# miemie2013/Pytorch-PPYOLO

Measured on AMD Instinct MI355X. Metric: images/sec PPYOLO R50-vd 608x608 bs=8, higher is better.
Workload: dtype f32; 1 GPU; PPYOLO ResNet50-vd (DCNv2, CoordConv, SPP) 608x608, 8 images per GPU, device-resident input -> padded detections; global_batch=8, parallelism=single GPU, hip_graph=True, tile_table=tuned_gfx950_f16x2.json

## Files before the change

### pytorch-ppyolo_amd/ppyolo_hip/csrc/conv_patch.hip

```cpp
#include "conv_shared.h"
#pragma clang fp contract(off)

#ifndef PPY_PATCH_ABL
#define PPY_PATCH_ABL 0
#endif

namespace {

constexpr unsigned PT_OOB = 0x80000000u;
constexpr int PT_TH = 8, PT_TW = 32, PT_PW = PT_TW + 2, PT_NPIX = (PT_TH + 2) * PT_PW;
constexpr int PT_PLANE = PT_NPIX * 64;
constexpr int PT_UNITS = PT_NPIX * 8, PT_NST = (PT_UNITS + 511) / 512;

constexpr int PM_ROWS = 3, PM_COLS = 15;

struct PatchArgs {
    ConvArgs c;
    int tiles_x, tiles_y, ntiles;
    int Hp, Wp;
};

template <int TN, bool BNS = false, bool MPOOL = false>
__global__ void __launch_bounds__(512, 1) conv3x3_patch_kernel(const PatchArgs q) {
    static_assert(!(BNS && MPOOL), "statistics of a tensor that is not stored");
    static_assert(PT_TH * PM_COLS * 32 * TN * 4 <= 2 * PT_PLANE, "the x-pooled rows fit the operand planes");
#if defined(__HIP_DEVICE_COMPILE__)
    const ConvArgs &p = q.c;
    constexpr int K = 32 * TN, WBYTES = 9 * 2 * K * 64;
    extern __shared__ __attribute__((aligned(16))) char smem_pt[];
    char *pl_hi = smem_pt, *pl_lo = smem_pt + PT_PLANE, *wl = smem_pt + 2 * PT_PLANE;
    const int tid = threadIdx.x, lane = tid & 63;
    const int wave = __builtin_amdgcn_readfirstlane(tid >> 6);
    float *sE = reinterpret_cast<float *>(smem_pt + 2 * PT_PLANE + WBYTES) + wave * (32 * LDS_LD);
    const __amdgpu_buffer_rsrc_t rx = __builtin_amdgcn_make_buffer_rsrc((void *)p.x, 0, PT_OOB, 0x00020000);
    const __amdgpu_buffer_rsrc_t ry = __builtin_amdgcn_make_buffer_rsrc((void *)p.y, 0, PT_OOB, 0x00020000);

    {
        const char *wb = reinterpret_cast<const char *>(p.wf16);
        const long long plane_bytes = (long long)K * 9 * 32 * 2;
        constexpr int WUNITS = 9 * 2 * K * 4, NWL = (WUNITS + 511) / 512;
        uintx4 wv[NWL];
#pragma unroll
        for (int i = 0; i < NWL; ++i) {
            const int u = min(tid + 512 * i, WUNITS - 1);
            const int slot = u & 3, row = u >> 2;
            const int k = row % K, tp = row / K, plane = tp & 1, tap = tp >> 1;
            wv[i] = *reinterpret_cast<const uintx4 *>(wb + plane * plane_bytes + ((long long)(tap * K + k) * 32) * 2 + slot * 16);
        }
#pragma unroll
        for (int i = 0; i < NWL; ++i) {
            const int u = tid + 512 * i;
            const int slot = u & 3, row = u >> 2;
            const int k = row % K;
            if (u < WUNITS) *reinterpret_cast<uintx4 *>(wl + row * 64 + ((slot ^ ((k >> 2) & 3)) << 4)) = wv[i];
        }
    }
    const int erow = lane >> 3, ec4 = (lane & 7) * 4;
    floatx4 sc[TN], sh[TN];
#pragma unroll
    for (int j = 0; j < TN; ++j) {
        sc[j] = *reinterpret_cast<const floatx4 *>(p.scale + j * 32 + ec4);
        sh[j] = *reinterpret_cast<const floatx4 *>(p.shift + j * 32 + ec4);
    }
#pragma unroll
    for (int j = 0; j < TN; ++j) asm volatile("" : "+v"(sc[j]), "+v"(sh[j]));

    int s_py[PT_NST], s_px[PT_NST];
#pragma unroll
    for (int i = 0; i < PT_NST; ++i) {
        const int pp = min((tid + 512 * i) >> 3, PT_NPIX - 1);
        s_py[i] = pp / PT_PW;
        s_px[i] = pp - s_py[i] * PT_PW;
    }
    uintx4 stg_a[PT_NST], stg_b[PT_NST];
#pragma unroll
    for (int i = 0; i < PT_NST; ++i) stg_a[i] = stg_b[i] = uintx4{0u, 0u, 0u, 0u};
    const int tiles_img = q.tiles_x * q.tiles_y;
    auto tile_of = [&](int t, int &n, int &y0, int &x0) {
        n = t / tiles_img;
        const int r = t - n * tiles_img, by = r / q.tiles_x;
        y0 = MPOOL ? 2 * PM_ROWS * by - 1 : by * PT_TH;
        x0 = MPOOL ? 2 * PM_COLS * (r - by * q.tiles_x) - 1 : (r - by * q.tiles_x) * PT_TW;
    };
    auto request = [&](int t, uintx4 (&stg)[PT_NST]) {
        int n, y0, x0;
        tile_of(max(t, 0), n, y0, x0);
        const bool live = t >= 0 && t < q.ntiles;
#pragma unroll
        for (int i = 0; i < PT_NST; ++i) {
            const int y = y0 - 1 + s_py[i], x = x0 - 1 + s_px[i];
            const bool ok = live && tid + 512 * i < PT_UNITS && (unsigned)y < (unsigned)p.H && (unsigned)x < (unsigned)p.W;
            const unsigned off = ok ? (unsigned)((n * p.H + y) * p.W + x) * (unsigned)(p.x_ld * 4) + (unsigned)((tid + 512 * i) & 7) * 16u : PT_OOB;
            if (PPY_PATCH_ABL != 4) stg[i] = __builtin_amdgcn_raw_buffer_load_b128(rx, (int)off, 0, 0);
        }
    };

    int sc_n = -1;
    float sa = 1.f, inv_sa = 1.f;
    int run_n = -1;
    float run_mx = 0.f;
    auto flush = [&](float mx, int n) {
        if (p.amax_out && n >= 0) {
#pragma unroll
            for (int o = 32; o > 0; o >>= 1) mx = fmaxf(mx, __shfl_xor(mx, o));
            if (lane == 0) amax_store(mx, p.amax_out, n, (int)blockIdx.x * 8 + wave);
        }
    };
    const float slope = p.act == PPY_ACT_RELU ? 0.f : (p.act == PPY_ACT_LEAKY ? 0.1f : 1.f);
    __syncthreads();
    const int stride = (int)gridDim.x;
    auto do_tile = [&](int t, uintx4 (&stg)[PT_NST]) {
        const bool live = t >= 0 && t < q.ntiles;
        int n, y0, x0;
        tile_of(live ? t : 0, n, y0, x0);
        if (live) {
        if (n != sc_n) {
            const float mx = conv_amax_in(p, n);
            const int e = (int)((__float_as_uint(mx) >> 23) & 0xffu);
            int f = 267 - e;
            f = f < 103 ? 103 : (f > 167 ? 167 : f);
            sa = __uint_as_float((unsigned)f << 23);
            inv_sa = __uint_as_float((unsigned)(254 - f) << 23);
            sc_n = n;
        }
        if (n != run_n) {
            flush(run_mx, run_n);
            run_n = n;
            run_mx = 0.f;
        }
#pragma unroll
        for (int i = 0; i < PT_NST; ++i) {
            const int u = tid + 512 * i;
            if (u < PT_UNITS && PPY_PATCH_ABL != 2) {
                const int pp = u >> 3, g = u & 7;
                const float x0f = __uint_as_float(stg[i][0]), x1f = __uint_as_float(stg[i][1]);
                const float x2f = __uint_as_float(stg[i][2]), x3f = __uint_as_float(stg[i][3]);
                const unsigned h0 = cvt_pk_f16(x0f * sa, x1f * sa), h1 = cvt_pk_f16(x2f * sa, x3f * sa);
                const unsigned l0 = cvt_pk_f16(fmaf(x0f, sa, -f16_lo(h0)), fmaf(x1f, sa, -f16_hi(h0)));
                const unsigned l1 = cvt_pk_f16(fmaf(x2f, sa, -f16_lo(h1)), fmaf(x3f, sa, -f16_hi(h1)));
                const int o = pp * 64 + (((g >> 1) ^ ((pp >> 2) & 3)) << 4) + (g & 1) * 8;
                typedef __attribute__((ext_vector_type(2))) unsigned uintx2;
                *reinterpret_cast<uintx2 *>(pl_hi + o) = uintx2{h0, h1};
                *reinterpret_cast<uintx2 *>(pl_lo + o) = uintx2{l0, l1};
            }
        }
        }
        asm volatile("s_waitcnt lgkmcnt(0)" ::: "memory");
        __builtin_amdgcn_s_barrier();
        request(t + 2 * stride, stg);

        floatx16 acc[TN];
#pragma unroll
        for (int j = 0; j < TN; ++j)
#pragma unroll
            for (int e = 0; e < 16; ++e) acc[j][e] = 0.f;
        const int tx = lane & 31, kh = lane >> 5;
        if (live && PPY_PATCH_ABL != 1 && (!MPOOL || wave < 2 * PM_ROWS + 1)) {
            struct Frag {
                uintx4 a0, a1, b0[TN], b1[TN];
            };
            Frag f[2];
            auto fetch = [&](Frag &fr, int g) {
                const int tap = g >> 1, s2 = g & 1;
                const int pp = (wave + tap / 3) * PT_PW + tx + tap % 3;
                const int ao = pp * 64 + (((2 * s2 + kh) ^ ((pp >> 2) & 3)) << 4);
                fr.a0 = *reinterpret_cast<const uintx4 *>(pl_hi + ao);
                fr.a1 = *reinterpret_cast<const uintx4 *>(pl_lo + ao);
#pragma unroll
                for (int j = 0; j < TN; ++j) {
                    const int k = j * 32 + tx;
                    const int bo = (((2 * s2 + kh) ^ ((k >> 2) & 3)) << 4);
                    fr.b0[j] = *reinterpret_cast<const uintx4 *>(wl + ((tap * 2 + 0) * K + k) * 64 + bo);
                    fr.b1[j] = *reinterpret_cast<const uintx4 *>(wl + ((tap * 2 + 1) * K + k) * 64 + bo);
                }
            };
            fetch(f[0], 0);
#pragma unroll
            for (int g = 0; g < 18; ++g) {
                if (g + 1 < 18 && PPY_PATCH_ABL != 5) fetch(f[(g + 1) & 1], g + 1);
                __builtin_amdgcn_sched_barrier(0);
                const Frag &c = f[PPY_PATCH_ABL == 5 ? 0 : g & 1];
#pragma unroll
                for (int j = 0; j < TN; ++j)
                    acc[j] = __builtin_amdgcn_mfma_f32_32x32x16_f16(__builtin_bit_cast(f16x8, c.a1), __builtin_bit_cast(f16x8, c.b0[j]), acc[j], 0, 0, 0);
#pragma unroll
                for (int j = 0; j < TN; ++j)
                    acc[j] = __builtin_amdgcn_mfma_f32_32x32x16_f16(__builtin_bit_cast(f16x8, c.a0), __builtin_bit_cast(f16x8, c.b1[j]), acc[j], 0, 0, 0);
#pragma unroll
                for (int j = 0; j < TN; ++j)
                    acc[j] = __builtin_amdgcn_mfma_f32_32x32x16_f16(__builtin_bit_cast(f16x8, c.a0), __builtin_bit_cast(f16x8, c.b0[j]), acc[j], 0, 0, 0);
                __builtin_amdgcn_sched_barrier(0);
            }
        }
        asm volatile("s_waitcnt lgkmcnt(0)" ::: "memory");
        __builtin_amdgcn_s_barrier();
        if (!live || PPY_PATCH_ABL == 3) return;

        const int y = y0 + wave;
        const bool row_ok = (unsigned)y < (unsigned)p.H;
        if constexpr (MPOOL) {
            float *xp = reinterpret_cast<float *>(smem_pt);
            constexpr int K4 = K / 4;
            if (wave < 2 * PM_ROWS + 1) {
#pragma unroll
                for (int j = 0; j < TN; ++j) {
#pragma unroll
                    for (int e = 0; e < 16; ++e) {
                        const int row = (e & 3) + 8 * (e >> 2) + 4 * (lane >> 5);
                        sE[row * LDS_LD + (lane & 31)] = acc[j][e];
                    }
                    __builtin_amdgcn_wave_barrier();
#pragma unroll
                    for (int u = 0; u < 4; ++u) {
                        floatx4 v = *reinterpret_cast<const floatx4 *>(sE + (erow + 8 * u) * LDS_LD + ec4);
#pragma unroll
                        for (int c = 0; c < 4; ++c) {
                            const float o = fmaf(v[c] * inv_sa, sc[j][c], sh[j][c]);
                            v[c] = o > 0.f ? o : o * slope + 0.0f;
                        }
                        const bool ok = row_ok && (unsigned)(x0 + erow + 8 * u) < (unsigned)p.W;
                        const float rmx = fmaxf(fmaxf(fabsf(v[0]), fabsf(v[1])), fmaxf(fabsf(v[2]), fabsf(v[3])));
                        run_mx = fmaxf(run_mx, ok ? rmx : 0.f);
                        if (!ok) v = floatx4{-3.402823466e38f, -3.402823466e38f, -3.402823466e38f, -3.402823466e38f};
                        *reinterpret_cast<floatx4 *>(sE + (erow + 8 * u) * LDS_LD + ec4) = v;
                    }
                    __builtin_amdgcn_wave_barrier();
#pragma unroll
                    for (int h = 0; h < 2; ++h) {
                        const int jx = erow + 8 * h;
                        if (jx < PM_COLS) {
                            const floatx4 a = *reinterpret_cast<const floatx4 *>(sE + (2 * jx) * LDS_LD + ec4);
                            const floatx4 b = *reinterpret_cast<const floatx4 *>(sE + (2 * jx + 1) * LDS_LD + ec4);
                            const floatx4 c = *reinterpret_cast<const floatx4 *>(sE + (2 * jx + 2) * LDS_LD + ec4);
                            floatx4 m;
#pragma unroll
                            for (int k = 0; k < 4; ++k) m[k] = fmaxf(fmaxf(a[k], b[k]), c[k]);
                            *reinterpret_cast<floatx4 *>(xp + (wave * PM_COLS + jx) * K + j * 32 + ec4) = m;
                        }
                    }
                    __builtin_amdgcn_wave_barrier();
                }
            }
            asm volatile("s_waitcnt lgkmcnt(0)" ::: "memory");
            __builtin_amdgcn_s_barrier();
            const int by = (y0 + 1) / (2 * PM_ROWS), bx = (x0 + 1) / (2 * PM_COLS);
#pragma unroll
            for (int it = 0; it < (PM_ROWS * PM_COLS * K4 + 511) / 512; ++it) {
                const int i = tid + 512 * it;
                const int r = i / (PM_COLS * K4), rem = i - r * (PM_COLS * K4);
                const int jx = rem / K4, c4 = rem - jx * K4;
                const int py = PM_ROWS * by + r, px = PM_COLS * bx + jx;
                const bool ok = i < PM_ROWS * PM_COLS * K4 && py < q.Hp && px < q.Wp;
                const int rr = ok ? r : 0, jj = ok ? jx : 0;
                const floatx4 a = *reinterpret_cast<const floatx4 *>(xp + ((2 * rr) * PM_COLS + jj) * K + c4 * 4);
                const floatx4 b = *reinterpret_cast<const floatx4 *>(xp + ((2 * rr + 1) * PM_COLS + jj) * K + c4 * 4);
                const floatx4 c = *reinterpret_cast<const floatx4 *>(xp + ((2 * rr + 2) * PM_COLS + jj) * K + c4 * 4);
                floatx4 m;
#pragma unroll
                for (int k = 0; k < 4; ++k) m[k] = fmaxf(fmaxf(a[k], b[k]), c[k]);
                const unsigned off = ok ? (unsigned)((n * q.Hp + py) * q.Wp + px) * (unsigned)(p.y_ld * 4) + (unsigned)c4 * 16u : PT_OOB;
                __builtin_amdgcn_raw_buffer_store_b128(__builtin_bit_cast(uintx4, m), ry, (int)off, 0, 0);
            }
            asm volatile("s_waitcnt lgkmcnt(0)" ::: "memory");
            __builtin_amdgcn_s_barrier();
            return;
        }
        if constexpr (BNS) {
            const int nv = row_ok ? min(max(p.W - x0, 0), 32) : 0;
            const float inv_f[1] = {inv_sa};
            tile_bn_stats<1, TN, 32, 32 * TN>(p, reinterpret_cast<const floatx16(&)[1][TN]>(acc), inv_f, p.M - nv, 0, 0, 0, lane, t * PT_TH + wave);
        }
        const unsigned rowbase = (unsigned)((n * p.H + y) * p.W + x0) * (unsigned)(p.y_ld * 4);
#pragma unroll
        for (int j = 0; j < TN; ++j) {
#pragma unroll
            for (int e = 0; e < 16; ++e) {
                const int row = (e & 3) + 8 * (e >> 2) + 4 * (lane >> 5);
                sE[row * LDS_LD + (lane & 31)] = acc[j][e];
            }
            __builtin_amdgcn_wave_barrier();
#pragma unroll
            for (int u = 0; u < 4; ++u) {
                floatx4 v = *reinterpret_cast<const floatx4 *>(sE + (erow + 8 * u) * LDS_LD + ec4);
#pragma unroll
                for (int c = 0; c < 4; ++c) {
                    const float o = fmaf(v[c] * inv_sa, sc[j][c], sh[j][c]);
                    v[c] = o > 0.f ? o : o * slope + 0.0f;
                }
                const bool ok = row_ok && x0 + erow + 8 * u < p.W;
                const float rmx = fmaxf(fmaxf(fabsf(v[0]), fabsf(v[1])), fmaxf(fabsf(v[2]), fabsf(v[3])));
                run_mx = fmaxf(run_mx, ok ? rmx : 0.f);
                const unsigned off = ok ? rowbase + (unsigned)(erow + 8 * u) * (unsigned)(p.y_ld * 4) + (unsigned)(j * 32 + ec4) * 4u : PT_OOB;
                __builtin_amdgcn_raw_buffer_store_b128(__builtin_bit_cast(uintx4, v), ry, (int)off, 0, 0);
            }
            __builtin_amdgcn_wave_barrier();
        }
    };
    for (int t = (int)blockIdx.x - 2 * stride; t < q.ntiles; t += 2 * stride) {
        do_tile(t, stg_a);
        do_tile(t + stride, stg_b);
    }
    flush(run_mx, run_n);
#endif
}

template <int TN, bool BNS = false, bool MPOOL = false>
int launch_patch(const PatchArgs &q, hipStream_t stream) {
    if constexpr (!BNS && !MPOOL) {
        if (q.c.bn_part) return launch_patch<TN, true>(q, stream);
    }
    auto k = conv3x3_patch_kernel<TN, BNS, MPOOL>;
    const size_t lds = (size_t)2 * PT_PLANE + (size_t)9 * 2 * 32 * TN * 64 + (size_t)8 * 32 * LDS_LD * sizeof(float);
    static PpyLdsAttr attr;
    if (ppy_lds_attr(attr, reinterpret_cast<const void *>(k), (int)lds) != PPY_OK) return PPY_ERR_LAUNCH;
    const int grid = q.ntiles < 256 ? q.ntiles : 256;
    hipLaunchKernelGGL(k, dim3(grid), dim3(512), lds, stream, q);
    return ppy_launch_status();
}

}

int ppy_patch_num_configs() { return 1; }

int ppy_patch_config_info(int local, ppy_conv_cfg_info *out) {
    if (local != 0) return PPY_ERR_BAD_ARG;
    *out = ppy_cfg_info(PPY_CFG_PATCH, local, PPY_CFG_OPERANDS_F16X2, 0, 0, 0, PPY_CFG_SPLITK_NONE, false, false, true);
    return PPY_OK;
}

int ppy_patch_dispatch(const ConvArgs &p, int local, hipStream_t stream) {
    if (local != 0) return PPY_ERR_BAD_ARG;
    if (p.R != 3 || p.S != 3 || p.stride != 1 || p.pad != 1 || p.C != 32 || (p.K != 32 && p.K != 64) || p.ups || p.posb || p.res)
        return PPY_ERR_BAD_ARG;
    if (!p.wf16 || ((uintptr_t)p.wf16 & 15) != 0 || !p.scale_f16 || !p.amax_in) return PPY_ERR_BAD_ARG;
    if (!vec_epilogue_ok(p) || ((uintptr_t)p.x & 15) != 0 || p.x_ld % 4 != 0) return PPY_ERR_BAD_ARG;
    const long long lim = 0x7FFFF000LL;
    if ((long long)p.M * p.x_ld * 4 >= lim || (long long)p.M * p.y_ld * 4 >= lim) return PPY_ERR_UNSUPPORTED;
    if (p.bn_part) {
        if (p.act != PPY_ACT_NONE) return PPY_ERR_UNSUPPORTED;
        if (p.N * ceil_div(p.W, PT_TW) * ceil_div(p.H, PT_TH) * PT_TH > p.bn_capacity) return PPY_ERR_WORKSPACE;
        if (p.bn_slices_host) *p.bn_slices_host = p.N * ceil_div(p.W, PT_TW) * ceil_div(p.H, PT_TH) * PT_TH;
    }
    PatchArgs q;
    q.c = p;
    q.c.scale = p.scale_f16;
    q.Hp = q.Wp = 0;
    q.tiles_x = ceil_div(p.W, PT_TW);
    q.tiles_y = ceil_div(p.H, PT_TH);
    q.ntiles = p.N * q.tiles_x * q.tiles_y;
    return p.K == 32 ? launch_patch<1>(q, stream) : launch_patch<2>(q, stream);
}

int ppy_patch_maxpool_dispatch(const ConvArgs &p, int Hp, int Wp, hipStream_t stream) {
    if (p.R != 3 || p.S != 3 || p.stride != 1 || p.pad != 1 || p.C != 32 || p.K != 64 || p.ups || p.posb || p.res || p.bn_part || p.xscale || p.yscale)
        return PPY_ERR_BAD_ARG;
    if (!p.wf16 || ((uintptr_t)p.wf16 & 15) != 0 || !p.scale_f16 || !p.amax_in) return PPY_ERR_BAD_ARG;
    if (((uintptr_t)p.x & 15) != 0 || p.x_ld % 4 != 0 || ((uintptr_t)p.y & 15) != 0 || p.y_ld % 4 != 0) return PPY_ERR_BAD_ARG;
    if (Hp != (p.H - 1) / 2 + 1 || Wp != (p.W - 1) / 2 + 1) return PPY_ERR_BAD_ARG;
    const long long lim = 0x7FFFF000LL;
    if ((long long)p.M * p.x_ld * 4 >= lim || (long long)p.N * Hp * Wp * p.y_ld * 4 >= lim) return PPY_ERR_UNSUPPORTED;
    PatchArgs q;
    q.c = p;
    q.c.scale = p.scale_f16;
    q.Hp = Hp;
    q.Wp = Wp;
    q.tiles_x = ceil_div(Wp, PM_COLS);
    q.tiles_y = ceil_div(Hp, PM_ROWS);
    q.ntiles = p.N * q.tiles_x * q.tiles_y;
    return launch_patch<2, false, true>(q, stream);
}
```

Before: 2465 images/s.

## Carry last conv row between pooled tiles to drop halo recompute in conv+maxpool

The fused 3x3 conv + maxpool kernel now gives each workgroup a contiguous column-major run of tiles, 4 pooled rows (8 conv rows) per tile, with one conv row per wave. The last conv row of each tile is kept in an extra LDS carry buffer and reused as the upper halo of the next tile, so the overlapping conv row is no longer recomputed. A run that starts mid-column first computes only that boundary row. This adds LDS use, serialises tiles within a workgroup, and adds an env override for the grid size.

```diff
diff --git a/pytorch-ppyolo_amd/ppyolo_hip/csrc/conv_patch.hip b/pytorch-ppyolo_amd/ppyolo_hip/csrc/conv_patch.hip
--- a/pytorch-ppyolo_amd/ppyolo_hip/csrc/conv_patch.hip
+++ b/pytorch-ppyolo_amd/ppyolo_hip/csrc/conv_patch.hip
@@ -12,12 +12,15 @@
 constexpr int PT_PLANE = PT_NPIX * 64;
 constexpr int PT_UNITS = PT_NPIX * 8, PT_NST = (PT_UNITS + 511) / 512;
 
-constexpr int PM_ROWS = 3, PM_COLS = 15;
+constexpr int PM_ROWS = 4, PM_COLS = 15;
+constexpr int PM_CARRY = PM_COLS * 64 * 4;
+static_assert(2 * PM_ROWS == PT_TH, "one conv row per wave: a pooled tile is the 8 x 32 tile of the plain form");
 
 struct PatchArgs {
     ConvArgs c;
     int tiles_x, tiles_y, ntiles;
     int Hp, Wp;
+    int wgs;
 };
 
 template <int TN, bool BNS = false, bool MPOOL = false>
@@ -76,20 +79,39 @@
 #pragma unroll
     for (int i = 0; i < PT_NST; ++i) stg_a[i] = stg_b[i] = uintx4{0u, 0u, 0u, 0u};
     const int tiles_img = q.tiles_x * q.tiles_y;
+    int m_first = 0, m_steps = 0;
+    bool m_pre = false;
+    if constexpr (MPOOL) {
+        const int G = (int)gridDim.x, g = (int)blockIdx.x;
+        const int lo = (int)((long long)q.ntiles * g / G), hi = (int)((long long)q.ntiles * (g + 1) / G);
+        m_pre = hi > lo && lo % q.tiles_y != 0;
+        m_first = lo - (m_pre ? 1 : 0);
+        m_steps = hi - m_first;
+    }
+    const int t_end = MPOOL ? m_steps : q.ntiles;
     auto tile_of = [&](int t, int &n, int &y0, int &x0) {
         n = t / tiles_img;
-        const int r = t - n * tiles_img, by = r / q.tiles_x;
-        y0 = MPOOL ? 2 * PM_ROWS * by - 1 : by * PT_TH;
-        x0 = MPOOL ? 2 * PM_COLS * (r - by * q.tiles_x) - 1 : (r - by * q.tiles_x) * PT_TW;
+        const int r = t - n * tiles_img;
+        if constexpr (MPOOL) {
+            const int bx = r / q.tiles_y;
+            y0 = (r - bx * q.tiles_y) * PT_TH;
+            x0 = 2 * PM_COLS * bx - 1;
+        } else {
+            const int by = r / q.tiles_x;
+            y0 = by * PT_TH;
+            x0 = (r - by * q.tiles_x) * PT_TW;
+        }
     };
     auto request = [&](int t, uintx4 (&stg)[PT_NST]) {
         int n, y0, x0;
-        tile_of(max(t, 0), n, y0, x0);
-        const bool live = t >= 0 && t < q.ntiles;
+        tile_of(m_first + max(t, 0), n, y0, x0);
+        const bool live = t >= 0 && t < t_end;
+        const bool pre = MPOOL && m_pre && t == 0;
 #pragma unroll
         for (int i = 0; i < PT_NST; ++i) {
             const int y = y0 - 1 + s_py[i], x = x0 - 1 + s_px[i];
-            const bool ok = live && tid + 512 * i < PT_UNITS && (unsigned)y < (unsigned)p.H && (unsigned)x < (unsigned)p.W;
+            const bool ok = live && tid + 512 * i < PT_UNITS && (unsigned)y < (unsigned)p.H && (unsigned)x < (unsigned)p.W &&
+                            (!pre || s_py[i] >= PT_TH - 1);
             const unsigned off = ok ? (unsigned)((n * p.H + y) * p.W + x) * (unsigned)(p.x_ld * 4) + (unsigned)((tid + 512 * i) & 7) * 16u : PT_OOB;
             if (PPY_PATCH_ABL != 4) stg[i] = __builtin_amdgcn_raw_buffer_load_b128(rx, (int)off, 0, 0);
         }
@@ -108,11 +130,12 @@
     };
     const float slope = p.act == PPY_ACT_RELU ? 0.f : (p.act == PPY_ACT_LEAKY ? 0.1f : 1.f);
     __syncthreads();
-    const int stride = (int)gridDim.x;
+    const int stride = MPOOL ? 1 : (int)gridDim.x;
     auto do_tile = [&](int t, uintx4 (&stg)[PT_NST]) {
-        const bool live = t >= 0 && t < q.ntiles;
+        const bool live = t >= 0 && t < t_end;
+        const bool pre = MPOOL && m_pre && t == 0;
         int n, y0, x0;
-        tile_of(live ? t : 0, n, y0, x0);
+        tile_of(live ? m_first + t : 0, n, y0, x0);
         if (live) {
         if (n != sc_n) {
             const float mx = conv_amax_in(p, n);
@@ -131,7 +154,7 @@
 #pragma unroll
         for (int i = 0; i < PT_NST; ++i) {
             const int u = tid + 512 * i;
-            if (u < PT_UNITS && PPY_PATCH_ABL != 2) {
+            if (u < PT_UNITS && PPY_PATCH_ABL != 2 && (!pre || s_py[i] >= PT_TH - 1)) {
                 const int pp = u >> 3, g = u & 7;
                 const float x0f = __uint_as_float(stg[i][0]), x1f = __uint_as_float(stg[i][1]);
                 const float x2f = __uint_as_float(stg[i][2]), x3f = __uint_as_float(stg[i][3]);
@@ -155,7 +178,7 @@
 #pragma unroll
             for (int e = 0; e < 16; ++e) acc[j][e] = 0.f;
         const int tx = lane & 31, kh = lane >> 5;
-        if (live && PPY_PATCH_ABL != 1 && (!MPOOL || wave < 2 * PM_ROWS + 1)) {
+        if (live && PPY_PATCH_ABL != 1 && (!pre || wave == PT_TH - 1)) {
             struct Frag {
                 uintx4 a0, a1, b0[TN], b1[TN];
             };
@@ -200,8 +223,9 @@
         const bool row_ok = (unsigned)y < (unsigned)p.H;
         if constexpr (MPOOL) {
             float *xp = reinterpret_cast<float *>(smem_pt);
+            float *carry = reinterpret_cast<float *>(smem_pt + 2 * PT_PLANE + WBYTES + 8 * 32 * LDS_LD * (int)sizeof(float));
             constexpr int K4 = K / 4;
-            if (wave < 2 * PM_ROWS + 1) {
+            if (!pre || wave == PT_TH - 1) {
 #pragma unroll
                 for (int j = 0; j < TN; ++j) {
 #pragma unroll
@@ -243,23 +267,32 @@
             }
             asm volatile("s_waitcnt lgkmcnt(0)" ::: "memory");
             __builtin_amdgcn_s_barrier();
-            const int by = (y0 + 1) / (2 * PM_ROWS), bx = (x0 + 1) / (2 * PM_COLS);
-#pragma unroll
-            for (int it = 0; it < (PM_ROWS * PM_COLS * K4 + 511) / 512; ++it) {
-                const int i = tid + 512 * it;
-                const int r = i / (PM_COLS * K4), rem = i - r * (PM_COLS * K4);
-                const int jx = rem / K4, c4 = rem - jx * K4;
-                const int py = PM_ROWS * by + r, px = PM_COLS * bx + jx;
-                const bool ok = i < PM_ROWS * PM_COLS * K4 && py < q.Hp && px < q.Wp;
-                const int rr = ok ? r : 0, jj = ok ? jx : 0;
-                const floatx4 a = *reinterpret_cast<const floatx4 *>(xp + ((2 * rr) * PM_COLS + jj) * K + c4 * 4);
-                const floatx4 b = *reinterpret_cast<const floatx4 *>(xp + ((2 * rr + 1) * PM_COLS + jj) * K + c4 * 4);
-                const floatx4 c = *reinterpret_cast<const floatx4 *>(xp + ((2 * rr + 2) * PM_COLS + jj) * K + c4 * 4);
-                floatx4 m;
-#pragma unroll
-                for (int k = 0; k < 4; ++k) m[k] = fmaxf(fmaxf(a[k], b[k]), c[k]);
-                const unsigned off = ok ? (unsigned)((n * q.Hp + py) * q.Wp + px) * (unsigned)(p.y_ld * 4) + (unsigned)c4 * 16u : PT_OOB;
-                __builtin_amdgcn_raw_buffer_store_b128(__builtin_bit_cast(uintx4, m), ry, (int)off, 0, 0);
+            const int b = y0 / PT_TH, bx = (x0 + 1) / (2 * PM_COLS);
+            if (pre) {
+                if (tid < PM_COLS * K4)
+                    *reinterpret_cast<floatx4 *>(carry + tid * 4) = *reinterpret_cast<const floatx4 *>(xp + (PT_TH - 1) * PM_COLS * K + tid * 4);
+            } else {
+#pragma unroll
+                for (int it = 0; it < (PM_ROWS * PM_COLS * K4 + 511) / 512; ++it) {
+                    const int i = tid + 512 * it;
+                    const int r = i / (PM_COLS * K4), rem = i - r * (PM_COLS * K4);
+                    const int jx = rem / K4, c4 = rem - jx * K4;
+                    const int py = PM_ROWS * b + r, px = PM_COLS * bx + jx;
+                    const bool in = i < PM_ROWS * PM_COLS * K4;
+                    const bool ok = in && py < q.Hp && px < q.Wp;
+                    const int rr = in ? r : 0, jj = in ? jx : 0;
+                    const float *up = in && rr == 0 && b > 0 ? carry + jj * K + c4 * 4 : xp + (max(2 * rr - 1, 0) * PM_COLS + jj) * K + c4 * 4;
+                    const floatx4 a = *reinterpret_cast<const floatx4 *>(up);
+                    const floatx4 b_ = *reinterpret_cast<const floatx4 *>(xp + ((2 * rr) * PM_COLS + jj) * K + c4 * 4);
+                    const floatx4 c = *reinterpret_cast<const floatx4 *>(xp + ((2 * rr + 1) * PM_COLS + jj) * K + c4 * 4);
+                    if (it == 0 && i < PM_COLS * K4)
+                        *reinterpret_cast<floatx4 *>(carry + i * 4) = *reinterpret_cast<const floatx4 *>(xp + (PT_TH - 1) * PM_COLS * K + i * 4);
+                    floatx4 m;
+#pragma unroll
+                    for (int k = 0; k < 4; ++k) m[k] = fmaxf(fmaxf(a[k], b_[k]), c[k]);
+                    const unsigned off = ok ? (unsigned)((n * q.Hp + py) * q.Wp + px) * (unsigned)(p.y_ld * 4) + (unsigned)c4 * 16u : PT_OOB;
+                    __builtin_amdgcn_raw_buffer_store_b128(__builtin_bit_cast(uintx4, m), ry, (int)off, 0, 0);
+                }
             }
             asm volatile("s_waitcnt lgkmcnt(0)" ::: "memory");
             __builtin_amdgcn_s_barrier();
@@ -296,7 +329,7 @@
             __builtin_amdgcn_wave_barrier();
         }
     };
-    for (int t = (int)blockIdx.x - 2 * stride; t < q.ntiles; t += 2 * stride) {
+    for (int t = (MPOOL ? 0 : (int)blockIdx.x) - 2 * stride; t < t_end; t += 2 * stride) {
         do_tile(t, stg_a);
         do_tile(t + stride, stg_b);
     }
@@ -310,10 +343,12 @@
         if (q.c.bn_part) return launch_patch<TN, true>(q, stream);
     }
     auto k = conv3x3_patch_kernel<TN, BNS, MPOOL>;
-    const size_t lds = (size_t)2 * PT_PLANE + (size_t)9 * 2 * 32 * TN * 64 + (size_t)8 * 32 * LDS_LD * sizeof(float);
+    const size_t lds = (size_t)2 * PT_PLANE + (size_t)9 * 2 * 32 * TN * 64 + (size_t)8 * 32 * LDS_LD * sizeof(float) + (MPOOL ? PM_CARRY : 0);
+    static_assert(!MPOOL || 2 * PT_PLANE + 9 * 2 * 32 * TN * 64 + 8 * 32 * LDS_LD * 4 + PM_CARRY <= PPY_LDS_MAX, "operand planes, weights, epilogue patches and the carried row in one CU's LDS");
     static PpyLdsAttr attr;
     if (ppy_lds_attr(attr, reinterpret_cast<const void *>(k), (int)lds) != PPY_OK) return PPY_ERR_LAUNCH;
-    const int grid = q.ntiles < 256 ? q.ntiles : 256;
+    const int cap = MPOOL ? q.wgs : 256;
+    const int grid = q.ntiles < cap ? q.ntiles : cap;
     hipLaunchKernelGGL(k, dim3(grid), dim3(512), lds, stream, q);
     return ppy_launch_status();
 }
@@ -344,7 +379,7 @@
     PatchArgs q;
     q.c = p;
     q.c.scale = p.scale_f16;
-    q.Hp = q.Wp = 0;
+    q.Hp = q.Wp = q.wgs = 0;
     q.tiles_x = ceil_div(p.W, PT_TW);
     q.tiles_y = ceil_div(p.H, PT_TH);
     q.ntiles = p.N * q.tiles_x * q.tiles_y;
@@ -367,5 +402,10 @@
     q.tiles_x = ceil_div(Wp, PM_COLS);
     q.tiles_y = ceil_div(Hp, PM_ROWS);
     q.ntiles = p.N * q.tiles_x * q.tiles_y;
+    q.wgs = 256;
+    if (const char *e = getenv("PPYOLO_HIP_PATCH_WGS")) {
+        const int v = atoi(e);
+        q.wgs = v < 1 ? 1 : (v > 256 ? 256 : v);
+    }
     return launch_patch<2, false, true>(q, stream);
 }
```

Measured after the change: 2483 images/s (median of 6 runs). No clear change (+0.7%).
